# AO33/HiC_Genome_Assembler

Measured on AMD Instinct MI355X. Metric: Part1+Part2 wall-clock (s) and bins/s on N x N contact map, higher is better.
Workload: dtype f64

## Files before the change

### hic_genome_assembler_amd/_lib.py

```python
from __future__ import annotations

import ctypes
import os

import numpy as np

_HERE = os.path.dirname(os.path.abspath(__file__))
LIB_PATH = os.environ.get("HICMI_LIB") or os.path.join(_HERE, "libhicmi.so")
_lib = None

c_i64 = ctypes.c_int64
c_dbl = ctypes.c_double
_vp = ctypes.c_void_p
_M64 = (1 << 64) - 1

SIGNATURES = {
    "hicmi_abi_version": (ctypes.c_int, []),
    "hicmi_last_error": (ctypes.c_char_p, []),
    "hicmi_device_count": (ctypes.c_int, [ctypes.POINTER(ctypes.c_int)]),
    "hicmi_create": (ctypes.c_int, [ctypes.c_int, ctypes.POINTER(_vp)]),
    "hicmi_destroy": (ctypes.c_int, [_vp]),
    "hicmi_stream": (ctypes.c_int, [_vp, ctypes.POINTER(_vp)]),
    "hicmi_synchronize": (ctypes.c_int, [_vp]),
    "hicmi_set_contacts_host": (ctypes.c_int, [_vp, _vp, c_i64]),
    "hicmi_set_contacts_host_f32": (ctypes.c_int, [_vp, _vp, c_i64]),
    "hicmi_set_contacts_device": (ctypes.c_int, [_vp, _vp, c_i64, c_i64]),
    "hicmi_contacts_device": (ctypes.c_int, [_vp, ctypes.POINTER(_vp), ctypes.POINTER(c_i64), ctypes.POINTER(c_i64)]),
    "hicmi_load_hicpro_matrix": (ctypes.c_int, [ctypes.c_char_p, _vp, c_i64, _vp, ctypes.c_int, ctypes.POINTER(c_i64)]),
    "hicmi_write_hicpro_matrix": (ctypes.c_int, [ctypes.c_char_p, _vp, c_i64, _vp, ctypes.c_int, ctypes.POINTER(c_i64)]),
    "hicmi_format_double": (ctypes.c_int, [c_dbl, ctypes.c_char_p, c_i64]),
    "hicmi_row_sums": (ctypes.c_int, [_vp, _vp, _vp]),
    "hicmi_set_row_shard": (ctypes.c_int, [_vp, c_i64, c_i64]),
    "hicmi_set_row_sums": (ctypes.c_int, [_vp, _vp, _vp]),
    "hicmi_compact": (ctypes.c_int, [_vp, _vp, c_i64]),
    "hicmi_rebin": (ctypes.c_int, [_vp, _vp, c_i64]),
    "hicmi_group_sums": (ctypes.c_int, [_vp, _vp, _vp, c_i64, c_i64, _vp, _vp]),
    "hicmi_junction_sums": (ctypes.c_int, [_vp, _vp, c_i64, _vp, c_i64, _vp]),
    "hicmi_get_contact_rows": (ctypes.c_int, [_vp, c_i64, c_i64, _vp]),
    "hicmi_ice_mask_rows": (ctypes.c_int, [_vp, _vp, c_i64]),
    "hicmi_ice_balance": (ctypes.c_int, [_vp, _vp, c_i64, c_dbl, _vp, ctypes.POINTER(c_i64), ctypes.POINTER(c_dbl)]),
    "hicmi_upgma": (ctypes.c_int, [_vp, _vp, _vp]),
    "hicmi_rank_matrix": (ctypes.c_int, [_vp, _vp]),
    "hicmi_presort_state": (ctypes.c_int, [_vp, _vp, _vp]),
    "hicmi_get_rank_rows": (ctypes.c_int, [_vp, c_i64, c_i64, ctypes.c_int, _vp]),
    "hicmi_get_similarity_row": (ctypes.c_int, [_vp, c_i64, _vp]),
    "hicmi_cut_scan": (ctypes.c_int, [_vp, c_i64, c_i64, c_dbl, _vp, _vp]),
    "hicmi_filter_scan": (ctypes.c_int, [_vp, c_i64, c_i64, c_i64, c_i64, c_dbl, _vp, _vp]),
    "hicmi_first_pass_cuts": (ctypes.c_int, [_vp, c_i64, c_i64, c_dbl, _vp, c_i64, _vp, _vp, c_i64, _vp]),
    "hicmi_filter_cuts": (ctypes.c_int, [_vp, _vp, c_i64, c_dbl, _vp, c_i64, _vp, _vp]),
    "hicmi_first_pass_cuts_multi": (ctypes.c_int, [_vp, c_i64, _vp, _vp, c_dbl, _vp, c_i64, _vp, _vp, c_i64, _vp]),
    "hicmi_filter_cuts_multi": (ctypes.c_int, [_vp, c_i64, _vp, _vp, _vp, _vp, c_i64, _vp, _vp]),
    "hicmi_hypergeom_decide": (ctypes.c_int, [c_i64, c_i64, c_i64, c_i64, c_dbl]),
    "hicmi_hypergeom_sf": (c_dbl, [c_i64, c_i64, c_i64, c_i64]),
    "hicmi_selftest_division": (ctypes.c_int, [_vp, ctypes.c_uint64, c_i64, ctypes.POINTER(ctypes.c_uint64)]),
    "hicmi_label_linkage": (ctypes.c_int, [_vp, c_i64, _vp]),
    "hicmi_leaf_order": (ctypes.c_int, [_vp, c_i64, _vp]),
    "hicmi_get_raw_merges": (ctypes.c_int, [_vp, _vp]),
    "hicmi_nnchain_stats": (ctypes.c_int, [_vp, _vp]),
    "hicmi_p2_select": (ctypes.c_int, [_vp, _vp, c_i64]),
    "hicmi_p2_total": (ctypes.c_int, [_vp, ctypes.POINTER(c_dbl)]),
    "hicmi_p2_score": (ctypes.c_int, [_vp, _vp, c_i64, c_i64, c_dbl, _vp]),
    "hicmi_p2_score_exact": (ctypes.c_int, [_vp, _vp, c_i64, c_i64, c_dbl, _vp]),
    "hicmi_p2_layout": (ctypes.c_int, [_vp, _vp, _vp, c_i64]),
    "hicmi_p2_set_arrangement": (ctypes.c_int, [_vp, _vp, _vp, c_i64]),
    "hicmi_p2_arrangement_total": (ctypes.c_int, [_vp, ctypes.POINTER(c_dbl)]),
    "hicmi_p2_arrangement_score": (ctypes.c_int, [_vp, c_dbl, ctypes.POINTER(c_dbl)]),
    "hicmi_p2_score_insertions": (ctypes.c_int, [_vp, ctypes.c_int32, c_dbl, _vp]),
    "hicmi_p2_window_tables": (ctypes.c_int, [_vp, c_i64, _vp, c_i64, _vp, c_i64]),
    "hicmi_p2_score_window": (ctypes.c_int, [_vp, c_i64, c_i64, _vp]),
    "hicmi_p2_decide_window": (ctypes.c_int, [_vp, c_i64, c_i64, c_dbl, c_dbl, c_dbl, ctypes.POINTER(c_i64),
                                              ctypes.POINTER(c_dbl), ctypes.POINTER(c_dbl)]),
    "hicmi_p2_window_shortlist": (ctypes.c_int, [_vp, c_i64, c_i64, c_i64, c_dbl, c_dbl, c_dbl, c_i64, _vp, _vp, _vp]),
    "hicmi_p2_decide_insertion": (ctypes.c_int, [_vp, _vp, _vp, c_i64, ctypes.c_int32, ctypes.c_int32,
                                                 ctypes.POINTER(c_i64), ctypes.POINTER(ctypes.c_int32),
                                                 ctypes.POINTER(c_dbl)]),
    "hicmi_p2_insert_all": (ctypes.c_int, [_vp, _vp, _vp, c_i64, _vp, c_i64, ctypes.POINTER(c_dbl)]),
    "hicmi_scan_valid_pairs": (ctypes.c_int, [ctypes.c_char_p, ctypes.c_char_p, _vp, c_i64, _vp, _vp, c_i64, ctypes.c_int,
                                              ctypes.POINTER(c_i64), ctypes.POINTER(c_i64), ctypes.POINTER(_vp)]),
    "hicmi_scan_fetch": (ctypes.c_int, [_vp, _vp, _vp, _vp]),
    "hicmi_parse_valid_pairs": (ctypes.c_int, [ctypes.c_char_p, ctypes.c_char_p, _vp, c_i64, _vp, ctypes.c_int, c_i64, c_i64,
                                               _vp, _vp, _vp, _vp, ctypes.POINTER(c_i64), ctypes.POINTER(c_i64), _vp]),
    "hicmi_map_begin": (ctypes.c_int, [_vp, _vp, c_i64, c_i64]),
    "hicmi_map_add_pairs": (ctypes.c_int, [_vp, _vp, _vp, _vp, _vp, c_i64]),
    "hicmi_map_finish": (ctypes.c_int, [_vp, ctypes.POINTER(c_i64)]),
    "hicmi_build_maps": (ctypes.c_int, [ctypes.c_char_p, ctypes.c_char_p, _vp, c_i64, _vp, c_i64, _vp, _vp, ctypes.c_int, _vp]),
    "hicmi_map_begin_lifted": (ctypes.c_int, [_vp, _vp, c_i64, _vp, _vp, _vp, _vp, c_i64, c_i64]),
# ... 545 lines not shown
        _check(self._lib.hicmi_nnchain_stats(self._h, _ptr(out)))
        return dict(merges=out[0], scans=out[1], scan_columns=out[2], cache_hits=out[3], retries=int(out[4]))

    def rank_matrix(self, order):
        order = np.ascontiguousarray(order, dtype=np.int32)
        if len(order) != self.n:
            raise ValueError("order must have n entries")
        _check(self._lib.hicmi_rank_matrix(self._h, _ptr(order)))

    def presort_state(self):
        st = ctypes.c_int(0)
        tied = c_i64(0)
        _check(self._lib.hicmi_presort_state(self._h, ctypes.byref(st), ctypes.byref(tied)))
        return st.value, int(tied.value)

    def rank_rows(self, row0=0, nrows=None, inverse=False):
        nrows = self.n - row0 if nrows is None else nrows
        out = np.empty((nrows, self.n), np.uint16)
        _check(self._lib.hicmi_get_rank_rows(self._h, row0, nrows, 1 if inverse else 0, _ptr(out)))
        return out

    def similarity_row(self, row):
        out = np.empty(self.n, np.float64)
        _check(self._lib.hicmi_get_similarity_row(self._h, row, _ptr(out)))
        return out

    def cut_scan(self, start, M, psig, want_x=False):
        cnt = self.n - start
        sig = np.empty(cnt, np.uint8)
        x = np.empty(cnt, np.int32) if want_x else None
        _check(self._lib.hicmi_cut_scan(self._h, start, M, psig, _ptr(x), _ptr(sig)))
        return (sig, x) if want_x else sig

    def filter_scan(self, start, c, n_rows, M, psig, want_x=False):
        sig = np.empty(n_rows, np.uint8)
        x = np.empty(n_rows, np.int32) if want_x else None
        _check(self._lib.hicmi_filter_scan(self._h, start, c, n_rows, M, psig, _ptr(x), _ptr(sig)))
        return (sig, x) if want_x else sig

    def first_pass_cuts(self, min_size, stop_ind, psig):
        cuts = np.empty(self.n, np.int32)
        mlog = np.empty((self.n, 2), np.int32)
        nc, nl = c_i64(0), c_i64(0)
        _check(self._lib.hicmi_first_pass_cuts(self._h, int(min_size), int(stop_ind), float(psig), _ptr(cuts), self.n,
                                               ctypes.byref(nc), _ptr(mlog), self.n, ctypes.byref(nl)))
        return [int(v) for v in cuts[:nc.value]], [(int(a), int(b)) for a, b in mlog[:nl.value]]

    def filter_cuts(self, cuts, psig):
        cuts = np.ascontiguousarray(cuts, dtype=np.int32)
        out = np.empty(self.n, np.int32)
        m, warned = c_i64(0), c_i64(0)
        _check(self._lib.hicmi_filter_cuts(self._h, _ptr(cuts), len(cuts), float(psig), _ptr(out), self.n,
                                           ctypes.byref(m), ctypes.byref(warned)))
        return [int(v) for v in out[:m.value]], int(warned.value)

    SCAN_MAX_SETS = 64

    def first_pass_cuts_multi(self, sets, psig):
        out = []
        n = self.n
        for c0 in range(0, len(sets), self.SCAN_MAX_SETS):
            part = sets[c0:c0 + self.SCAN_MAX_SETS]
            k = len(part)
            ms = np.array([int(a) for a, _b in part], np.int64)
            si = np.array([int(b) for _a, b in part], np.int64)
            cuts = np.empty((k, n), np.int32)
# ... 511 lines not shown
```

### hic_genome_assembler_amd/csrc/api.hip

```cpp
#include <hip/hip_runtime.h>

#include <algorithm>
#include <cmath>
#include <cstdarg>
#include <climits>
#include <cstdio>
#include <cstdlib>
#include <cstring>
#include <numeric>
#include <string>
#include <unordered_map>
#include <functional>
#include <chrono>
#include <vector>

#include "../../include/hicmi.h"
#include "hicmi_internal.h"
#include "devbuf.h"
#include "hyper.h"

using namespace hicmi;

static thread_local std::string g_err;

// ... 1994 lines not shown
        c->cached_start = start;
    }
    return finish_scan(c, cnt, 0, 0, M, psig, x_out, sig_out, t0);
}

int hicmi_filter_scan(hicmi_ctx* c, int64_t start, int64_t cut, int64_t n_rows, int64_t M, double psig,
                      int32_t* x_out, uint8_t* sig_out)
{
    if (!c) return fail(HICMI_EINVAL, "NULL context");
    if (!c->have_rank) return fail(HICMI_EINVAL, "hicmi_rank_matrix has not run");
    const int64_t n = c->n;
    if (start < 0 || start >= n || cut < start || cut >= n || n_rows < 0 || start + n_rows > n)
        return fail(HICMI_EINVAL, "filter scan arguments out of range");
    HIPCHK(hipSetDevice(c->device));
    int rc = ensure_scan_buffers(c);
    if (rc) return rc;
    c->cached_start = -1;
    const int64_t st = c->shard_stride;
    const int64_t t0 = ((c->shard_first - start) % st + st) % st;
    if (st > 1) HIPCHK(hipMemsetAsync(c->d_x, 0, sizeof(int32_t) * (size_t)n_rows, c->stream));
    {
        Timed t(c, F_CUT_COUNT, 2.0 * (double)n_rows * (double)(cut - start + 1) / (double)st);
        if (t0 < n_rows)
            launch_cut_count(c->dRank, c->ldr, (int)(start + t0), (int)(n_rows - t0), (int)start, 1, (int)cut, c->d_x + t0, (int)st,
                             c->stream);
    }
    HIPCHK(hipGetLastError());
    return finish_scan(c, n_rows, 1, cut - start, M, psig, x_out, sig_out, t0);
}

double hicmi_hypergeom_sf(int64_t x, int64_t M, int64_t n, int64_t N) { return hypergeom_sf_ge(x, M, n, N); }
int hicmi_hypergeom_decide(int64_t x, int64_t M, int64_t n, int64_t N, double psig) { return hypergeom_decide(x, M, n, N, psig); }

static_assert(SCAN_MAX_SETS == HICMI_SCAN_MAX_SETS, "hicmi.h and the kernels disagree on the set cap");

struct ScanMulti {
    ScanState* st; int32_t *x, *cuts, *mlog, *alt, *seg, *seg_x; uint8_t *sig, *filt, *prev;
};

static int ensure_scan_multi(hicmi_ctx* c, int sets, ScanMulti& m)
{
    const size_t n = (size_t)c->n, S = (size_t)sets;
    const size_t head = (sizeof(ScanState) * SCAN_MAX_SETS + 255) & ~(size_t)255;
    const size_t bytes = head + S * n * (sizeof(int32_t) * 9 + 3) + 64;
    int rc = ensure(c->d_scan_multi, (int64_t)bytes);
    if (rc) return rc;
    unsigned char* b = c->d_scan_multi;
    m.st = reinterpret_cast<ScanState*>(b);
    m.x = reinterpret_cast<int32_t*>(b + head);
    m.cuts = m.x + S * n; m.mlog = m.cuts + S * n; m.alt = m.mlog + 2 * S * n; m.seg = m.alt + S * n; m.seg_x = m.seg + 3 * S * n;
    m.sig = reinterpret_cast<uint8_t*>(m.seg_x + S * n); m.filt = m.sig + S * n; m.prev = m.filt + S * n;
    return HICMI_OK;
}

static int scan_share()
{
    const char* e = getenv("HICMI_SCAN_SHARE");
    return e && !strcmp(e, "0") ? 0 : 1;
}

static int run_scan_multi(hicmi_ctx* c, std::vector<ScanState>& h, const ScanMulti& m, const std::vector<int64_t>& max_scans,
                          const std::function<void(int)>& enqueue)
{
    const size_t S = h.size();
    int rc = upload(c, m.st, h.data(), sizeof(ScanState) * S);
    if (rc) return rc;
// ... 2344 lines not shown
```

### hic_genome_assembler_amd/csrc/hicmi_internal.h

```cpp
#pragma once
#include <hip/hip_runtime.h>
#include <stdint.h>

#include <atomic>
#include <functional>

#include "liftmap.h"
#include "span.h"
#include "split.h"

namespace hicmi {

inline void ensure_dynamic_lds(const void* func, std::atomic<int>& have, size_t bytes)
{
    if ((int)bytes > have.load(std::memory_order_relaxed)) {
        (void)hipFuncSetAttribute(func, hipFuncAttributeMaxDynamicSharedMemorySize, (int)bytes);
        have.store((int)bytes, std::memory_order_relaxed);
    }
}

static constexpr int SERIAL_BATCH = 16;

__device__ __forceinline__ double serial_sum_lds(const double* t, int from, int to, double acc)
{
// ... 102 lines not shown
    int xcc = -1;
    int test_late = 0, test_diverge = 0, test_rollcall = 0;
};
NNChainOptions nnchain_options(int probed_xcc);
int nnchain_probe_xcc(hipStream_t s);
int launch_nnchain(double* W, double* W2, int64_t ldw, int n, int* chain, double* zraw, void* workspace, const NNChainOptions& o,
                   int fallback, hipStream_t s, const std::function<void()>& after_first_rowmin = nullptr);
void launch_selftest_division(unsigned long long seed, int blocks, int iters, unsigned long long* d_mismatches, hipStream_t s);
const int* nnchain_state_ptr(void* workspace);
const unsigned long long* nnchain_prof_ptr(void* workspace);
void launch_cut_count(const uint16_t* rank, int64_t ldr, int row0, int nrows, int lo, int mode, int cparam,
                      int32_t* x_out, int row_step, hipStream_t s);
void launch_hyper_flags(const int32_t* x, int nrows, int mode, int L_fixed, int64_t M, double psig, uint8_t* sig,
                        int own_first, int own_step, hipStream_t s);

struct ScanState {
    int done;
    int mode;
    int start, cut, n_rows, recount;
    long long M;
    double psig;
    int min_size, stop_ind, loop_count, n_cuts, n_log, scans;
    int MD, n_alt, alt_off, f_i, f_keep_from, f_noise, f_round, f_max_rounds, f_warned;
    int pad;
    unsigned long long bytes;
};
static constexpr int SCAN_MAX_SETS = 64;
void launch_first_pass_multi_pairs(const uint16_t* rank, int64_t ldr, int n, int n_sets, ScanState* st, int32_t* x, uint8_t* sig,
                                   double psig0, int share, int32_t* cuts, int32_t* mlog, int log_cap, int pairs, hipStream_t s);
void launch_filter_multi_pairs(const uint16_t* rank, int64_t ldr, int n, int max_rows, int n_sets, ScanState* st, int32_t* x,
                               uint8_t* sig, double psig0, int share, int32_t* alt, uint8_t* filt, uint8_t* prev,
                               int32_t* seg, int32_t* seg_x, int pairs, hipStream_t s);

#if defined(__HIPCC__)
template <int M>
__device__ __forceinline__ uint32_t xor_lane(uint32_t v, int lane)
{
    if constexpr (M == 1) return (uint32_t)__builtin_amdgcn_mov_dpp((int)v, 0xB1, 0xf, 0xf, true);
    else if constexpr (M == 2) return (uint32_t)__builtin_amdgcn_mov_dpp((int)v, 0x4E, 0xf, 0xf, true);
    else if constexpr (M == 4) {
        const int t = __builtin_amdgcn_mov_dpp((int)v, 0x141, 0xf, 0xf, true);
        return (uint32_t)__builtin_amdgcn_mov_dpp(t, 0x1B, 0xf, 0xf, true);
    } else if constexpr (M == 8) {
        const int t = __builtin_amdgcn_mov_dpp((int)v, 0x140, 0xf, 0xf, true);
        return (uint32_t)__builtin_amdgcn_mov_dpp(t, 0x141, 0xf, 0xf, true);
    } else if constexpr (M == 16) {
        const auto r = __builtin_amdgcn_permlane16_swap(v, v, false, false);
        return (lane & 16) ? r[0] : r[1];
    } else {
        static_assert(M == 32, "xor_lane: M must be 1, 2, 4, 8, 16 or 32");
        const auto r = __builtin_amdgcn_permlane32_swap(v, v, false, false);
        return (lane & 32) ? r[0] : r[1];
    }
}
#endif

int  sort_padded_size(int n);
int  sort_workgroups(int n);
size_t sort_scratch_bytes(int n);
struct SortExtras {
    const int32_t* row_list = nullptr; int n_list = 0;
    uint8_t* tie_flag = nullptr; unsigned* tie_count = nullptr; unsigned tie_limit = 0;
    uint16_t* tie_bits = nullptr; int64_t ld_bits = 0;
    int max_workgroups = 0;
    int avoid_xcc = -1; unsigned* row_counter = nullptr;
};
// ... 344 lines not shown
```

### hic_genome_assembler_amd/csrc/hyper.h

```cpp
#pragma once
#include <math.h>
#include <stdint.h>

#if defined(__HIPCC__)
#define HICMI_HD __host__ __device__ inline
#else
#define HICMI_HD inline
#endif

namespace hicmi {

HICMI_HD double stirlerr(double n)
{
    const double S0 = 0.083333333333333333333;
    const double S1 = 0.00277777777777777777778;
    const double S2 = 0.00079365079365079365079365;
    const double S3 = 0.000595238095238095238095238;
    const double S4 = 0.0008417508417508417508417508;
    if (n <= 15.0) {
        switch ((int)n) {
        case 0: return 0.0;
        case 1: return 0.08106146679532725821967026;
        case 2: return 0.04134069595540929409382208;
        case 3: return 0.02767792568499833914878929;
// ... 6 lines not shown
        case 10: return 0.008330563433362871256469319;
        case 11: return 0.007573675487951840794972024;
        case 12: return 0.006942840107209529865664153;
        case 13: return 0.006408994188004207068439631;
        case 14: return 0.005951370112758847735624416;
        default: return 0.00555473355196280137103869;
        }
    }
    double nn = n * n;
    if (n > 500.0) return (S0 - S1 / nn) / n;
    if (n > 80.0) return (S0 - (S1 - S2 / nn) / nn) / n;
    if (n > 35.0) return (S0 - (S1 - (S2 - S3 / nn) / nn) / nn) / n;
    return (S0 - (S1 - (S2 - (S3 - S4 / nn) / nn) / nn) / nn) / n;
}

HICMI_HD double bd0(double x, double np)
{
    if (fabs(x - np) < 0.1 * (x + np)) {
        double v = (x - np) / (x + np);
        double s = (x - np) * v;
        double ej = 2.0 * x * v;
        v = v * v;
        for (int j = 1; j < 1000; j++) {
            ej *= v;
            double s1 = s + ej / (double)((j << 1) + 1);
            if (s1 == s) return s1;
            s = s1;
        }
        return s;
    }
    return x * log(x / np) + np - x;
}

HICMI_HD double dbinom_raw(double x, double n, double p, double q)
{
    if (p == 0.0) return x == 0.0 ? 1.0 : 0.0;
    if (q == 0.0) return x == n ? 1.0 : 0.0;
    if (x == 0.0) {
        if (n == 0.0) return 1.0;
        double lc = (p < 0.1) ? -bd0(n, n * q) - n * p : n * log(q);
        return exp(lc);
    }
    if (x == n) {
        double lc = (q < 0.1) ? -bd0(n, n * p) - n * q : n * log(p);
        return exp(lc);
    }
    if (x < 0.0 || x > n) return 0.0;
    double lc = stirlerr(n) - stirlerr(x) - stirlerr(n - x) - bd0(x, n * p) - bd0(n - x, n * q);
    double lf = 1.837877066409345483560659  + log(x) + log1p(-x / n);
    return exp(lc - 0.5 * lf);
}

HICMI_HD double dhyper(double k, double r, double b, double d)
{
    if (d < k || r < k || d - k > b || k < 0.0) return 0.0;
    if (d == 0.0) return k == 0.0 ? 1.0 : 0.0;
    double p = d / (r + b), q = (r + b - d) / (r + b);
    double p1 = dbinom_raw(k, r, p, q);
    double p2 = dbinom_raw(d - k, b, p, q);
    double p3 = dbinom_raw(d, r + b, p, q);
    return p1 * p2 / p3;
}

HICMI_HD double hypergeom_sf_ge(int64_t x, int64_t M, int64_t n, int64_t N)
{
    if (!(M > 0 && n >= 0 && N >= 0 && n <= M && N <= M)) return NAN;
    int64_t lo = N - (M - n); if (lo < 0) lo = 0;
    int64_t hi = n < N ? n : N;
    if (x <= lo) return 1.0;
    if (x > hi) return 0.0;
    const double r = (double)n, b = (double)(M - n), d = (double)N;
    int64_t mode = (int64_t)floor(((double)(n + 1) * (double)(N + 1)) / (double)(M + 2));
    if (x > mode) {
        double term = dhyper((double)x, r, b, d);
        double sum = term;
        for (int64_t k = x; k < hi; k++) {
            double num = (double)(n - k) * (double)(N - k);
            double den = (double)(k + 1) * (double)(M - n - N + k + 1);
            term *= num / den;
            double s1 = sum + term;
            if (s1 == sum) break;
            sum = s1;
        }
        return sum > 1.0 ? 1.0 : sum;
    }
    double term = dhyper((double)(x - 1), r, b, d);
    double sum = term;
    for (int64_t k = x - 1; k > lo; k--) {
        double num = (double)k * (double)(M - n - N + k);
        double den = (double)(n - k + 1) * (double)(N - k + 1);
        term *= num / den;
        double s1 = sum + term;
        if (s1 == sum) break;
        sum = s1;
    }
    double sf = 1.0 - sum;
    return sf < 0.0 ? 0.0 : sf;
}

HICMI_HD int hypergeom_decide(int64_t x, int64_t M, int64_t n, int64_t N, double psig)
{
    if (!(M > 0 && n >= 0 && N >= 0 && n <= M && N <= M)) return -1;
    int64_t lo = N - (M - n); if (lo < 0) lo = 0;
    int64_t hi = n < N ? n : N;
    if (x <= lo) return 1.0 < psig ? 1 : 0;
    if (x > hi) return 0.0 < psig ? 1 : 0;
    const double r = (double)n, b = (double)(M - n), d = (double)N;
    const double below = psig * (1.0 - 1e-9), above = psig * (1.0 + 1e-9);
    int64_t mode = (int64_t)floor(((double)(n + 1) * (double)(N + 1)) / (double)(M + 2));
    if (x > mode) {
        double term = dhyper((double)x, r, b, d);
        double sum = term;
        if (!(sum < psig)) return sum != sum ? -1 : 0;
        for (int64_t k = x; k < hi; k++) {
            double num = (double)(n - k) * (double)(N - k);
            double den = (double)(k + 1) * (double)(M - n - N + k + 1);
            const double ratio = num / den;
            term *= ratio;
            double s1 = sum + term;
            if (s1 == sum) break;
            sum = s1;
            if (!(sum < psig)) return 0;
            if (ratio < 1.0 && term * ratio < (below - sum) * (1.0 - ratio)) return 1;
        }
        return (sum > 1.0 ? 1.0 : sum) < psig ? 1 : 0;
    }
    double term = dhyper((double)(x - 1), r, b, d);
    double sum = term;
    if (1.0 - sum < psig) return 1;
    for (int64_t k = x - 1; k > lo; k--) {
        double num = (double)k * (double)(M - n - N + k);
        double den = (double)(n - k + 1) * (double)(N - k + 1);
        const double ratio = num / den;
        term *= ratio;
        double s1 = sum + term;
        if (s1 == sum) break;
        sum = s1;
        if (1.0 - sum < psig) return 1;
        if (ratio <= 0.5 && 1.0 - (sum + term) > above) return 0;
    }
    double sf = 1.0 - sum;
    if (sf < 0.0) sf = 0.0;
    return sf < psig ? 1 : 0;
}

}
```

### hic_genome_assembler_amd/csrc/k_part1_scan.hip

```cpp
#include "hicmi_internal.h"
#include "hyper.h"

namespace hicmi {

__device__ __forceinline__ int row_count_partial(const uint16_t* __restrict__ r, int lo, int end, int thr, int tid)
{
    int cnt = 0;
    int body0 = (lo + 7) & ~7;
    if (body0 > end) body0 = end;
    const int body1 = body0 + ((end - body0) & ~7);
    for (int j = lo + tid; j < body0; j += 256) cnt += (int)r[j] < thr;
    for (int j = body0 + tid * 8; j < body1; j += 256 * 8) {
        uint4 q = *reinterpret_cast<const uint4*>(r + j);
        cnt += (int)(q.x & 0xffffu) < thr; cnt += (int)(q.x >> 16) < thr;
        cnt += (int)(q.y & 0xffffu) < thr; cnt += (int)(q.y >> 16) < thr;
        cnt += (int)(q.z & 0xffffu) < thr; cnt += (int)(q.z >> 16) < thr;
        cnt += (int)(q.w & 0xffffu) < thr; cnt += (int)(q.w >> 16) < thr;
    }
    for (int j = body1 + tid; j < end; j += 256) cnt += (int)r[j] < thr;
    return cnt;
}

__device__ __forceinline__ uint8_t row_flag(int mode, int total, long long M, int t, int thr, double psig)
{
    if (mode == 0) return hypergeom_decide((int64_t)total, M, (int64_t)t, (int64_t)t, psig) == 0 ? 0 : 1;
    return hypergeom_decide((int64_t)total, M, (int64_t)thr, (int64_t)thr, psig) == 1 ? 1 : 0;
}

__global__ __launch_bounds__(256) void k_cut_rows(const uint16_t* __restrict__ rank, int64_t ldr, int n,
                                                  const ScanState* __restrict__ st, int32_t* __restrict__ x,
                                                  uint8_t* __restrict__ sig, double psig)
{
    __shared__ int s_part[4];
    if (st->done) return;
    const int mode = st->mode, lo = st->start, t = blockIdx.x;
    const int rows = mode == 0 ? n - lo : st->n_rows;
    if (t >= rows) return;
    const int tid = threadIdx.x;
    if (mode == 0 && t == 0) { if (tid == 0) sig[0] = 0; return; }
    const int i = lo + t;
    const int hi = mode == 0 ? i : st->cut;
    const int thr = hi - lo;
    int total;
    if (st->recount) {
        int cnt = row_count_partial(rank + (int64_t)i * ldr, lo, hi + 1, thr, tid);
#pragma unroll
        for (int off = 32; off >= 1; off >>= 1) cnt += __shfl_xor(cnt, off, 64);
        if ((tid & 63) == 0) s_part[tid >> 6] = cnt;
        __syncthreads();
        if (tid != 0) return;
        total = s_part[0] + s_part[1] + s_part[2] + s_part[3];
        x[t] = total;
    } else {
        if (tid != 0) return;
        total = x[t];
    }
    sig[t] = row_flag(mode, total, st->M, t, thr, psig);
}

__device__ __forceinline__ void first_pass_decide(int n, ScanState* __restrict__ st, const uint8_t* __restrict__ sig,
                                                  int32_t* __restrict__ cuts, int32_t* __restrict__ mlog, int log_cap)
{
    __shared__ int s_sum[16];
    __shared__ int s_first;
    __shared__ int s_go;
    if (st->done) return;
    const int tid = threadIdx.x;
    const int start = st->start, cnt = n - start, h = st->min_size;
    int part = 0;
    for (int e = tid; e < cnt; e += 1024) part += sig[e];
#pragma unroll
    for (int off = 32; off >= 1; off >>= 1) part += __shfl_xor(part, off, 64);
    if ((tid & 63) == 0) s_sum[tid >> 6] = part;
    if (tid == 0) s_first = 0x7fffffff;
    __syncthreads();
    if (tid == 0) {
        int total = 0;
        for (int w = 0; w < 16; w++) total += s_sum[w];
        int go = 1;
        st->scans++;
        if (st->recount) { const unsigned long long m = (unsigned long long)(cnt - 1); st->bytes += m * (m + 3); }
        st->loop_count++;
        if ((double)total / (double)cnt >= .9) {
            const int64_t morg = st->M;
            st->M = morg - start;
            if (st->n_log < log_cap) { mlog[2 * st->n_log] = (int32_t)morg; mlog[2 * st->n_log + 1] = (int32_t)st->M; }
            st->n_log++;
            if (st->loop_count < 5) { go = 0; st->recount = 0; }
        }
        s_go = go;
// ... 263 lines not shown
```

### include/hicmi.h

```cpp
#ifndef HICMI_H
#define HICMI_H

#include <stdint.h>

#ifdef __cplusplus
extern "C" {
#endif

#define HICMI_ABI_VERSION 1

#define HICMI_OK            0
#define HICMI_EINVAL       -1
#define HICMI_EHIP         -2
#define HICMI_ENOMEM       -3
#define HICMI_ESTATE       -4
#define HICMI_EUNSUPPORTED -5

typedef struct hicmi_ctx hicmi_ctx;

int         hicmi_abi_version(void);
const char *hicmi_last_error(void);
int         hicmi_device_count(int *count);

int hicmi_create(int device, hicmi_ctx **out);
// ... 18 lines not shown
int hicmi_set_row_shard(hicmi_ctx *ctx, int64_t first, int64_t stride);
int hicmi_set_row_sums(hicmi_ctx *ctx, const double *np_sum, const double *seq_sum);

int hicmi_compact(hicmi_ctx *ctx, const int32_t *keep, int64_t n_keep);

int hicmi_rebin(hicmi_ctx *ctx, const int32_t *group_start, int64_t m);

int hicmi_upgma(hicmi_ctx *ctx, double *Z_out, int32_t *leaves_out);

int hicmi_rank_matrix(hicmi_ctx *ctx, const int32_t *order);
int hicmi_presort_state(hicmi_ctx *ctx, int *state_out, int64_t *tied_rows_out);
int hicmi_get_rank_rows(hicmi_ctx *ctx, int64_t row0, int64_t nrows, int inverse, uint16_t *out);
int hicmi_get_similarity_row(hicmi_ctx *ctx, int64_t row, double *out);

int hicmi_cut_scan(hicmi_ctx *ctx, int64_t start, int64_t M, double psig, int32_t *x_out, uint8_t *sig_out);

int hicmi_filter_scan(hicmi_ctx *ctx, int64_t start, int64_t c, int64_t n_rows, int64_t M, double psig,
                      int32_t *x_out, uint8_t *sig_out);

int hicmi_first_pass_cuts(hicmi_ctx *ctx, int64_t min_size, int64_t stop_ind, double psig, int32_t *cuts_out,
                          int64_t cuts_cap, int64_t *n_cuts_out, int32_t *m_log_out, int64_t log_cap, int64_t *n_log_out);
int hicmi_filter_cuts(hicmi_ctx *ctx, const int32_t *cuts_in, int64_t n_in, double psig, int32_t *cuts_out,
                      int64_t cuts_cap, int64_t *n_out, int64_t *warned_out);

#define HICMI_SCAN_MAX_SETS 64
int hicmi_first_pass_cuts_multi(hicmi_ctx *ctx, int64_t n_sets, const int64_t *min_size, const int64_t *stop_ind, double psig,
                                int32_t *cuts_out, int64_t cuts_cap, int64_t *n_cuts_out, int32_t *m_log_out, int64_t log_cap,
                                int64_t *n_log_out);
int hicmi_filter_cuts_multi(hicmi_ctx *ctx, int64_t n_sets, const int64_t *cand_off, const int32_t *cuts_in, const double *psig,
                            int32_t *cuts_out, int64_t cuts_cap, int64_t *n_out, int64_t *warned_out);

double hicmi_hypergeom_sf(int64_t x, int64_t M, int64_t n, int64_t N);
int hicmi_hypergeom_decide(int64_t x, int64_t M, int64_t n, int64_t N, double psig);

int hicmi_label_linkage(const double *Zraw, int64_t n, double *Z_out);
int hicmi_leaf_order(const double *Z, int64_t n, int32_t *leaves_out);
int hicmi_selftest_division(hicmi_ctx *ctx, uint64_t seed, int64_t samples, uint64_t *mismatches_out);
int hicmi_get_raw_merges(hicmi_ctx *ctx, double *Zraw_out);
int hicmi_nnchain_stats(hicmi_ctx *ctx, double *out6);

int hicmi_p2_select(hicmi_ctx *ctx, const int32_t *sel, int64_t n);
int hicmi_p2_total(hicmi_ctx *ctx, double *total_out);
int hicmi_p2_score(hicmi_ctx *ctx, const int32_t *perms, int64_t n_cand, int64_t n_used, double total,
                   double *scores_out);
int hicmi_p2_score_exact(hicmi_ctx *ctx, const int32_t *perms, int64_t n_cand, int64_t n_used, double total,
                         double *scores_out);

int hicmi_p2_layout(hicmi_ctx *ctx, const int32_t *scaf_start, const int32_t *scaf_len, int64_t n_scaf);
int hicmi_p2_set_arrangement(hicmi_ctx *ctx, const int32_t *ids, const uint8_t *rev, int64_t S);
int hicmi_p2_arrangement_total(hicmi_ctx *ctx, double *total_out);
int hicmi_p2_arrangement_score(hicmi_ctx *ctx, double total, double *score_out);
int hicmi_p2_score_insertions(hicmi_ctx *ctx, int32_t new_id, double total, double *scores_out);
int hicmi_p2_window_tables(hicmi_ctx *ctx, int64_t k, const int8_t *orders, int64_t n_orders,
                           const uint8_t *orients, int64_t n_orients);
int hicmi_p2_score_window(hicmi_ctx *ctx, int64_t first, int64_t k, double *delta_out);

int hicmi_p2_decide_window(hicmi_ctx *ctx, int64_t first, int64_t k, double total, double floor, double cur_fast,
                           int64_t *pick_out, double *best_out, double *pick_fast_out);
int hicmi_p2_window_shortlist(hicmi_ctx *ctx, int64_t first, int64_t count, int64_t k, double total, double floor,
                              double cur_fast, int64_t cap, int64_t *n_near_out, int64_t *idx_out, double *fast_out);
int hicmi_p2_decide_insertion(hicmi_ctx *ctx, const int32_t *ids, const uint8_t *rev, int64_t S, int32_t new_id,
                              int32_t new_rev_now, int64_t *gap_out, int32_t *rev_out, double *best_out);

int hicmi_p2_insert_all(hicmi_ctx *ctx, int32_t *ids, uint8_t *rev, int64_t S0, const int32_t *new_ids, int64_t n_new,
                        double *best_out);
int hicmi_p2_scan_pass(hicmi_ctx *ctx, int32_t *ids, uint8_t *rev, int64_t S, int64_t k, double total, double *best_io,
// ... 142 lines not shown
```

Before: 123,500.

## Evaluate hypergeometric decision with a full wavefront instead of one thread

The per-row hypergeometric significance test in k_cut_rows now runs across a whole 64-lane wavefront instead of a single thread. The 15 stirlerr/bd0/log pieces of the three binomial densities are computed in parallel lanes and gathered with shuffles, and tail ratios are precomputed 64 at a time and then consumed serially via readlane. This targets the serial latency of the single-thread hypergeometric tail loop. It also adds a standalone device API for batch decisions, and cross-lane reads plus different evaluation order risk small numerical differences and extra overhead when tails are short.

```diff
diff --git a/hic_genome_assembler_amd/_lib.py b/hic_genome_assembler_amd/_lib.py
--- a/hic_genome_assembler_amd/_lib.py
+++ b/hic_genome_assembler_amd/_lib.py
@@ -52,6 +52,7 @@
     "hicmi_filter_cuts_multi": (ctypes.c_int, [_vp, c_i64, _vp, _vp, _vp, _vp, c_i64, _vp, _vp]),
     "hicmi_hypergeom_decide": (ctypes.c_int, [c_i64, c_i64, c_i64, c_i64, c_dbl]),
     "hicmi_hypergeom_sf": (c_dbl, [c_i64, c_i64, c_i64, c_i64]),
+    "hicmi_hypergeom_decide_device": (ctypes.c_int, [_vp, c_i64, _vp, _vp, _vp, _vp, c_dbl, _vp]),
     "hicmi_selftest_division": (ctypes.c_int, [_vp, ctypes.c_uint64, c_i64, ctypes.POINTER(ctypes.c_uint64)]),
     "hicmi_label_linkage": (ctypes.c_int, [_vp, c_i64, _vp]),
     "hicmi_leaf_order": (ctypes.c_int, [_vp, c_i64, _vp]),
@@ -663,6 +664,14 @@
         _check(self._lib.hicmi_cut_scan(self._h, start, M, psig, _ptr(x), _ptr(sig)))
         return (sig, x) if want_x else sig
 
+    def hypergeom_decide_device(self, x, M, n, N, psig):
+        args = [np.ascontiguousarray(v, np.int64) for v in (x, M, n, N)]
+        if len({a.shape for a in args}) != 1 or args[0].ndim != 1:
+            raise ValueError("x, M, n, N: one-dimensional arrays of one length")
+        out = np.empty(len(args[0]), np.int32)
+        _check(self._lib.hicmi_hypergeom_decide_device(self._h, len(out), *[_ptr(a) for a in args], float(psig), _ptr(out)))
+        return out
+
     def filter_scan(self, start, c, n_rows, M, psig, want_x=False):
         sig = np.empty(n_rows, np.uint8)
         x = np.empty(n_rows, np.int32) if want_x else None
diff --git a/hic_genome_assembler_amd/csrc/api.hip b/hic_genome_assembler_amd/csrc/api.hip
--- a/hic_genome_assembler_amd/csrc/api.hip
+++ b/hic_genome_assembler_amd/csrc/api.hip
@@ -2050,6 +2050,30 @@
 double hicmi_hypergeom_sf(int64_t x, int64_t M, int64_t n, int64_t N) { return hypergeom_sf_ge(x, M, n, N); }
 int hicmi_hypergeom_decide(int64_t x, int64_t M, int64_t n, int64_t N, double psig) { return hypergeom_decide(x, M, n, N, psig); }
 
+int hicmi_hypergeom_decide_device(hicmi_ctx* c, int64_t count, const int64_t* x, const int64_t* M, const int64_t* n, const int64_t* N,
+                                  double psig, int32_t* out)
+{
+    if (!c) return fail(HICMI_EINVAL, "null context");
+    if (count < 0 || count > (1 << 24)) return fail(HICMI_EINVAL, "tuple count out of range");
+    if (count == 0) return HICMI_OK;
+    if (!x || !M || !n || !N || !out) return fail(HICMI_EINVAL, "null argument");
+    HIPCHK(hipSetDevice(c->device));
+    DevBuf<int64_t> d_args;
+    DevBuf<int32_t> d_out;
+    size_t failed = 0;
+    if (reserve_all(&failed, d_args, 4 * count, d_out, count) != hipSuccess)
+        return fail(HICMI_ENOMEM, "hipMalloc of %zu bytes failed", failed);
+    const int64_t* src[4] = {x, M, n, N};
+    for (int k = 0; k < 4; k++)
+        HIPCHK(hipMemcpyAsync(d_args.get() + k * count, src[k], sizeof(int64_t) * (size_t)count, hipMemcpyHostToDevice, c->stream));
+    launch_hypergeom_decide_wave((int)count, d_args.get(), d_args.get() + count, d_args.get() + 2 * count, d_args.get() + 3 * count,
+                                 psig, d_out.get(), c->stream);
+    HIPCHK(hipGetLastError());
+    HIPCHK(hipMemcpyAsync(out, d_out.get(), sizeof(int32_t) * (size_t)count, hipMemcpyDeviceToHost, c->stream));
+    HIPCHK(hipStreamSynchronize(c->stream));
+    return HICMI_OK;
+}
+
 static_assert(SCAN_MAX_SETS == HICMI_SCAN_MAX_SETS, "hicmi.h and the kernels disagree on the set cap");
 
 struct ScanMulti {
diff --git a/hic_genome_assembler_amd/csrc/hicmi_internal.h b/hic_genome_assembler_amd/csrc/hicmi_internal.h
--- a/hic_genome_assembler_amd/csrc/hicmi_internal.h
+++ b/hic_genome_assembler_amd/csrc/hicmi_internal.h
@@ -158,6 +158,9 @@
                                uint8_t* sig, double psig0, int share, int32_t* alt, uint8_t* filt, uint8_t* prev,
                                int32_t* seg, int32_t* seg_x, int pairs, hipStream_t s);
 
+void launch_hypergeom_decide_wave(int count, const int64_t* x, const int64_t* M, const int64_t* n, const int64_t* N, double psig,
+                                  int32_t* out, hipStream_t s);
+
 #if defined(__HIPCC__)
 template <int M>
 __device__ __forceinline__ uint32_t xor_lane(uint32_t v, int lane)
diff --git a/hic_genome_assembler_amd/csrc/hyper.h b/hic_genome_assembler_amd/csrc/hyper.h
--- a/hic_genome_assembler_amd/csrc/hyper.h
+++ b/hic_genome_assembler_amd/csrc/hyper.h
@@ -62,34 +62,114 @@
     return x * log(x / np) + np - x;
 }
 
-HICMI_HD double dbinom_raw(double x, double n, double p, double q)
+enum { PIECE_NONE = 0, PIECE_STIRLERR = 1, PIECE_BD0 = 2, PIECE_LOG = 3, PIECE_LF = 4 };
+static constexpr int DBINOM_PIECES = 6;
+struct Piece { int kind; double a, b; };
+
+HICMI_HD Piece dbinom_piece(int j, double x, double n, double p, double q)
+{
+    Piece pc = {PIECE_NONE, 0.0, 0.0};
+    if (p == 0.0 || q == 0.0) return pc;
+    if (x == 0.0) {
+        if (n == 0.0 || j != 3) return pc;
+        if (p < 0.1) { pc.kind = PIECE_BD0; pc.a = n; pc.b = n * q; } else { pc.kind = PIECE_LOG; pc.a = q; }
+        return pc;
+    }
+    if (x == n) {
+        if (j != 3) return pc;
+        if (q < 0.1) { pc.kind = PIECE_BD0; pc.a = n; pc.b = n * p; } else { pc.kind = PIECE_LOG; pc.a = p; }
+        return pc;
+    }
+    if (x < 0.0 || x > n) return pc;
+    switch (j) {
+    case 0: pc.kind = PIECE_STIRLERR; pc.a = n; break;
+    case 1: pc.kind = PIECE_STIRLERR; pc.a = x; break;
+    case 2: pc.kind = PIECE_STIRLERR; pc.a = n - x; break;
+    case 3: pc.kind = PIECE_BD0; pc.a = x; pc.b = n * p; break;
+    case 4: pc.kind = PIECE_BD0; pc.a = n - x; pc.b = n * q; break;
+    default: pc.kind = PIECE_LF; pc.a = x; pc.b = n; break;
+    }
+    return pc;
+}
+
+HICMI_HD double piece_lf(double x, double n) { return 1.837877066409345483560659  + log(x) + log1p(-x / n); }
+
+HICMI_HD double piece_eval(const Piece pc)
+{
+    switch (pc.kind) {
+    case PIECE_STIRLERR: return stirlerr(pc.a);
+    case PIECE_BD0: return bd0(pc.a, pc.b);
+    case PIECE_LOG: return log(pc.a);
+    case PIECE_LF: return piece_lf(pc.a, pc.b);
+    default: return 0.0;
+    }
+}
+
+HICMI_HD double dbinom_combine(double x, double n, double p, double q, const double* v)
 {
     if (p == 0.0) return x == 0.0 ? 1.0 : 0.0;
     if (q == 0.0) return x == n ? 1.0 : 0.0;
     if (x == 0.0) {
         if (n == 0.0) return 1.0;
-        double lc = (p < 0.1) ? -bd0(n, n * q) - n * p : n * log(q);
+        double lc = (p < 0.1) ? -v[3] - n * p : n * v[3];
         return exp(lc);
     }
     if (x == n) {
-        double lc = (q < 0.1) ? -bd0(n, n * p) - n * q : n * log(p);
+        double lc = (q < 0.1) ? -v[3] - n * q : n * v[3];
         return exp(lc);
     }
     if (x < 0.0 || x > n) return 0.0;
-    double lc = stirlerr(n) - stirlerr(x) - stirlerr(n - x) - bd0(x, n * p) - bd0(n - x, n * q);
-    double lf = 1.837877066409345483560659  + log(x) + log1p(-x / n);
-    return exp(lc - 0.5 * lf);
-}
-
+    double lc = v[0] - v[1] - v[2] - v[3] - v[4];
+    return exp(lc - 0.5 * v[5]);
+}
+
+HICMI_HD double dbinom_raw(double x, double n, double p, double q)
+{
+    double v[DBINOM_PIECES];
+#if defined(__HIPCC__)
+#pragma unroll
+#endif
+    for (int j = 0; j < DBINOM_PIECES; j++) v[j] = piece_eval(dbinom_piece(j, x, n, p, q));
+    return dbinom_combine(x, n, p, q, v);
+}
+
+HICMI_HD bool dhyper_is_const(double k, double r, double b, double d) { return d < k || r < k || d - k > b || k < 0.0 || d == 0.0; }
+HICMI_HD double dhyper_const(double k, double r, double b, double d)
+{
+    if (d < k || r < k || d - k > b || k < 0.0) return 0.0;
+    return k == 0.0 ? 1.0 : 0.0;
+}
+HICMI_HD void dhyper_binom_args(int i, double k, double r, double b, double d, double* x, double* n)
+{
+    if (i == 0) { *x = k; *n = r; } else if (i == 1) { *x = d - k; *n = b; } else { *x = d; *n = r + b; }
+}
 HICMI_HD double dhyper(double k, double r, double b, double d)
 {
-    if (d < k || r < k || d - k > b || k < 0.0) return 0.0;
-    if (d == 0.0) return k == 0.0 ? 1.0 : 0.0;
-    double p = d / (r + b), q = (r + b - d) / (r + b);
-    double p1 = dbinom_raw(k, r, p, q);
-    double p2 = dbinom_raw(d - k, b, p, q);
-    double p3 = dbinom_raw(d, r + b, p, q);
-    return p1 * p2 / p3;
+    if (dhyper_is_const(k, r, b, d)) return dhyper_const(k, r, b, d);
+    const double p = d / (r + b), q = (r + b - d) / (r + b);
+    double pb[3];
+#if defined(__HIPCC__)
+#pragma unroll
+#endif
+    for (int i = 0; i < 3; i++) {
+        double x, n;
+        dhyper_binom_args(i, k, r, b, d, &x, &n);
+        pb[i] = dbinom_raw(x, n, p, q);
+    }
+    return pb[0] * pb[1] / pb[2];
+}
+
+HICMI_HD double tail_ratio_up(int64_t k, int64_t M, int64_t n, int64_t N)
+{
+    double num = (double)(n - k) * (double)(N - k);
+    double den = (double)(k + 1) * (double)(M - n - N + k + 1);
+    return num / den;
+}
+HICMI_HD double tail_ratio_down(int64_t k, int64_t M, int64_t n, int64_t N)
+{
+    double num = (double)k * (double)(M - n - N + k);
+    double den = (double)(n - k + 1) * (double)(N - k + 1);
+    return num / den;
 }
 
 HICMI_HD double hypergeom_sf_ge(int64_t x, int64_t M, int64_t n, int64_t N)
@@ -105,9 +185,7 @@
         double term = dhyper((double)x, r, b, d);
         double sum = term;
         for (int64_t k = x; k < hi; k++) {
-            double num = (double)(n - k) * (double)(N - k);
-            double den = (double)(k + 1) * (double)(M - n - N + k + 1);
-            term *= num / den;
+            term *= tail_ratio_up(k, M, n, N);
             double s1 = sum + term;
             if (s1 == sum) break;
             sum = s1;
@@ -143,9 +221,7 @@
         double sum = term;
         if (!(sum < psig)) return sum != sum ? -1 : 0;
         for (int64_t k = x; k < hi; k++) {
-            double num = (double)(n - k) * (double)(N - k);
-            double den = (double)(k + 1) * (double)(M - n - N + k + 1);
-            const double ratio = num / den;
+            const double ratio = tail_ratio_up(k, M, n, N);
             term *= ratio;
             double s1 = sum + term;
             if (s1 == sum) break;
diff --git a/hic_genome_assembler_amd/csrc/hyper_wave.h b/hic_genome_assembler_amd/csrc/hyper_wave.h
--- /dev/null
+++ b/hic_genome_assembler_amd/csrc/hyper_wave.h
@@ -0,0 +1,110 @@
+#pragma once
+#include "hyper.h"
+
+#if defined(__HIPCC__)
+namespace hicmi {
+
+__device__ __forceinline__ double wave_read(double v, int src)
+{
+    const long long bits = __double_as_longlong(v);
+    const int lo = __builtin_amdgcn_readlane((int)(bits & 0xffffffffll), src);
+    const int hi = __builtin_amdgcn_readlane((int)(bits >> 32), src);
+    return __longlong_as_double((long long)(((unsigned long long)(unsigned int)hi << 32) | (unsigned long long)(unsigned int)lo));
+}
+__device__ __forceinline__ double dhyper_wave(double k, double r, double b, double d, int g)
+{
+    if (dhyper_is_const(k, r, b, d)) return dhyper_const(k, r, b, d);
+    const double p = d / (r + b), q = (r + b - d) / (r + b);
+    Piece pc = {PIECE_NONE, 0.0, 0.0};
+    if (g < 15) {
+        const int i = g < 9 ? g / 3 : (g - 9) >> 1, j = g < 9 ? g % 3 : 3 + ((g - 9) & 1);
+        double x, n;
+        dhyper_binom_args(i, k, r, b, d, &x, &n);
+        pc = dbinom_piece(j, x, n, p, q);
+    }
+    const double v1 = piece_eval(pc);
+    const int i = g < 2 ? g : 2;
+    double x, n;
+    dhyper_binom_args(i, k, r, b, d, &x, &n);
+    Piece pf = {PIECE_NONE, 0.0, 0.0};
+    if (g < 3) pf = dbinom_piece(5, x, n, p, q);
+    double v[DBINOM_PIECES];
+    v[0] = __shfl(v1, 3 * i, 64);
+    v[1] = __shfl(v1, 3 * i + 1, 64);
+    v[2] = __shfl(v1, 3 * i + 2, 64);
+    v[3] = __shfl(v1, 9 + 2 * i, 64);
+    v[4] = __shfl(v1, 10 + 2 * i, 64);
+    v[5] = pf.kind == PIECE_LF ? piece_lf(pf.a, pf.b) : 0.0;
+    const double pb = dbinom_combine(x, n, p, q, v);
+    const double p1 = wave_read(pb, 0), p2 = wave_read(pb, 1), p3 = wave_read(pb, 2);
+    return p1 * p2 / p3;
+}
+
+enum { TAIL_ON = 0, TAIL_SAME = 1, TAIL_REACHED = 2, TAIL_SETTLED = 3 };
+template <bool UP>
+__device__ __forceinline__ int tail_test(double ratio, double term, double sum, double s1, double psig, double edge)
+{
+    if (s1 == sum) return TAIL_SAME;
+    if constexpr (UP) {
+        if (!(s1 < psig)) return TAIL_REACHED;
+        if (ratio < 1.0 && term * ratio < (edge - s1) * (1.0 - ratio)) return TAIL_SETTLED;
+    } else {
+        if (1.0 - s1 < psig) return TAIL_REACHED;
+        if (ratio <= 0.5 && 1.0 - (s1 + term) > edge) return TAIL_SETTLED;
+    }
+    return TAIL_ON;
+}
+template <bool UP>
+__device__ __forceinline__ int tail_wave(double& term, double& sum, int64_t k_first, int64_t n_terms, int64_t M, int64_t n,
+                                         int64_t N, double psig, double edge, int lane)
+{
+    for (int64_t done = 0; done < n_terms; done += 64) {
+        const int cnt = n_terms - done < 64 ? (int)(n_terms - done) : 64;
+        const int64_t kl = UP ? k_first + done + lane : k_first - done - lane;
+        const double mine = lane < cnt ? (UP ? tail_ratio_up(kl, M, n, N) : tail_ratio_down(kl, M, n, N)) : 0.0;
+        for (int i = 0; i < cnt; i++) {
+            const double ratio = wave_read(mine, i);
+            term *= ratio;
+            const double s1 = sum + term;
+            const int why = tail_test<UP>(ratio, term, sum, s1, psig, edge);
+            if (why == TAIL_SAME) return why;
+            sum = s1;
+            if (why != TAIL_ON) return why;
+        }
+    }
+    return TAIL_ON;
+}
+
+__device__ __forceinline__ int hypergeom_decide_wave(int64_t x, int64_t M, int64_t n, int64_t N, double psig)
+{
+    const int lane = (int)(threadIdx.x & 63);
+    if (!(M > 0 && n >= 0 && N >= 0 && n <= M && N <= M)) return -1;
+    int64_t lo = N - (M - n); if (lo < 0) lo = 0;
+    int64_t hi = n < N ? n : N;
+    if (x <= lo) return 1.0 < psig ? 1 : 0;
+    if (x > hi) return 0.0 < psig ? 1 : 0;
+    const double r = (double)n, b = (double)(M - n), d = (double)N;
+    const double below = psig * (1.0 - 1e-9), above = psig * (1.0 + 1e-9);
+    int64_t mode = (int64_t)floor(((double)(n + 1) * (double)(N + 1)) / (double)(M + 2));
+    if (x > mode) {
+        double term = dhyper_wave((double)x, r, b, d, lane);
+        double sum = term;
+        if (!(sum < psig)) return sum != sum ? -1 : 0;
+        const int why = tail_wave<true>(term, sum, x, hi - x, M, n, N, psig, below, lane);
+        if (why == TAIL_REACHED) return 0;
+        if (why == TAIL_SETTLED) return 1;
+        return (sum > 1.0 ? 1.0 : sum) < psig ? 1 : 0;
+    }
+    double term = dhyper_wave((double)(x - 1), r, b, d, lane);
+    double sum = term;
+    if (1.0 - sum < psig) return 1;
+    const int why = tail_wave<false>(term, sum, x - 1, x - 1 - lo, M, n, N, psig, above, lane);
+    if (why == TAIL_REACHED) return 1;
+    if (why == TAIL_SETTLED) return 0;
+    double sf = 1.0 - sum;
+    if (sf < 0.0) sf = 0.0;
+    return sf < psig ? 1 : 0;
+}
+
+}
+#endif
diff --git a/hic_genome_assembler_amd/csrc/k_part1_scan.hip b/hic_genome_assembler_amd/csrc/k_part1_scan.hip
--- a/hic_genome_assembler_amd/csrc/k_part1_scan.hip
+++ b/hic_genome_assembler_amd/csrc/k_part1_scan.hip
@@ -1,5 +1,6 @@
 #include "hicmi_internal.h"
 #include "hyper.h"
+#include "hyper_wave.h"
 
 namespace hicmi {
 
@@ -25,6 +26,12 @@
 {
     if (mode == 0) return hypergeom_decide((int64_t)total, M, (int64_t)t, (int64_t)t, psig) == 0 ? 0 : 1;
     return hypergeom_decide((int64_t)total, M, (int64_t)thr, (int64_t)thr, psig) == 1 ? 1 : 0;
+}
+
+__device__ __forceinline__ uint8_t row_flag_wave(int mode, int total, long long M, int t, int thr, double psig)
+{
+    if (mode == 0) return hypergeom_decide_wave((int64_t)total, M, (int64_t)t, (int64_t)t, psig) == 0 ? 0 : 1;
+    return hypergeom_decide_wave((int64_t)total, M, (int64_t)thr, (int64_t)thr, psig) == 1 ? 1 : 0;
 }
 
 __global__ __launch_bounds__(256) void k_cut_rows(const uint16_t* __restrict__ rank, int64_t ldr, int n,
@@ -48,14 +55,32 @@
         for (int off = 32; off >= 1; off >>= 1) cnt += __shfl_xor(cnt, off, 64);
         if ((tid & 63) == 0) s_part[tid >> 6] = cnt;
         __syncthreads();
-        if (tid != 0) return;
+        if (tid >= 64) return;
         total = s_part[0] + s_part[1] + s_part[2] + s_part[3];
-        x[t] = total;
+        if (tid == 0) x[t] = total;
     } else {
-        if (tid != 0) return;
+        if (tid >= 64) return;
         total = x[t];
     }
-    sig[t] = row_flag(mode, total, st->M, t, thr, psig);
+    const uint8_t flag = row_flag_wave(mode, __builtin_amdgcn_readfirstlane(total), st->M, t, thr, psig);
+    if (tid == 0) sig[t] = flag;
+}
+
+__global__ __launch_bounds__(256) void k_hypergeom_decide_wave(int count, const int64_t* __restrict__ x, const int64_t* __restrict__ M,
+                                                               const int64_t* __restrict__ n, const int64_t* __restrict__ N,
+                                                               double psig, int32_t* __restrict__ out)
+{
+    const int w = (int)blockIdx.x * 4 + __builtin_amdgcn_readfirstlane((int)(threadIdx.x >> 6));
+    if (w >= count) return;
+    const int dec = hypergeom_decide_wave(x[w], M[w], n[w], N[w], psig);
+    if ((threadIdx.x & 63) == 0) out[w] = dec;
+}
+
+void launch_hypergeom_decide_wave(int count, const int64_t* x, const int64_t* M, const int64_t* n, const int64_t* N, double psig,
+                                  int32_t* out, hipStream_t s)
+{
+    if (count <= 0) return;
+    hipLaunchKernelGGL(k_hypergeom_decide_wave, dim3((count + 3) / 4), dim3(256), 0, s, count, x, M, n, N, psig, out);
 }
 
 __device__ __forceinline__ void first_pass_decide(int n, ScanState* __restrict__ st, const uint8_t* __restrict__ sig,
diff --git a/include/hicmi.h b/include/hicmi.h
--- a/include/hicmi.h
+++ b/include/hicmi.h
@@ -74,6 +74,8 @@
 
 double hicmi_hypergeom_sf(int64_t x, int64_t M, int64_t n, int64_t N);
 int hicmi_hypergeom_decide(int64_t x, int64_t M, int64_t n, int64_t N, double psig);
+int hicmi_hypergeom_decide_device(hicmi_ctx* ctx, int64_t count, const int64_t* x, const int64_t* M, const int64_t* n,
+                                  const int64_t* N, double psig, int32_t* out);
 
 int hicmi_label_linkage(const double *Zraw, int64_t n, double *Z_out);
 int hicmi_leaf_order(const double *Z, int64_t n, int32_t *leaves_out);
```

Measured after the change: 119,300. 0.966x the previous value.
